# freewym/espresso

Measured on AMD Instinct MI355X. Metric: audio-hours/sec training (LibriSpeech Conformer-12 + CTC), higher is better.
Workload: dtype bf16; 1 GPU; LibriSpeech 960h Conformer-12 + CTC update step, <=26000 frames & <=24 utts per GPU, V=5004, on-GPU fbank+CMVN+SpecAugment, dropout 0.1, clip 2.0, Adam; parallelism=dp1

## Files before the change

### espresso_amd/csrc/conv_igemm.hip

```cpp
#include <hip/hip_runtime.h>

#include "gemm_common.h"

namespace {

typedef const __attribute__((address_space(1))) void* gptr_t;
typedef __attribute__((address_space(3))) void* lptr_t;

struct ConvGatherArgs {
  const bf16_t* src;
  const bf16_t* W;
  bf16_t* out;
  const float* bias;
  double* stats;
  const bf16_t* zero;
  int RB, RT, RF;
  int ST, SF, SC;
  int at, af;
  int ntaps;
  int bt[9], bf[9], koff[9];
  int N;
  long ldw;
  int OT, OF, ot_mul, ot_add, of_mul, of_add;
};

template <int BN_>
__global__ __launch_bounds__(256, 2) void conv_gather_kernel(const ConvGatherArgs a) {
  constexpr int BM_ = 128, NST = 2;
  constexpr int NJ = BN_ / 32;
  constexpr int A_BYTES = BM_ * ROW_BYTES, STAGE = A_BYTES + BN_ * ROW_BYTES;
  constexpr int NA = BM_ / 32, NB = BN_ / 32;
  extern __shared__ __attribute__((aligned(16))) char dsm[];
  const int tid = threadIdx.x, lane = tid & 63, wave = tid >> 6;
  const int wm = wave >> 1, wcol = (wave & 1) * (BN_ / 2);
  const uint32_t M = (uint32_t)a.RB * a.RT * a.RF;
  const uint32_t m0 = blockIdx.x * BM_;
  const int cpt = a.SC / BK;
  const int nk = a.ntaps * cpt;

  int rowb[NA], rowt[NA], rowf[NA];
  int cs[NA];
#pragma unroll
  for (int i = 0; i < NA; ++i) {
    const int r = (wave + 4 * i) * 8 + (lane >> 3);
    cs[i] = (lane & 7) ^ (r & 7) ^ ((r >> 4) & 7);
    const uint32_t p = m0 + r;
    if (p < M) {
      const uint32_t q = p / (uint32_t)a.RF, b = q / (uint32_t)a.RT;
      const int rf = (int)(p - q * a.RF), rt = (int)(q - b * a.RT);
      rowb[i] = (int)b * a.ST;
      rowt[i] = rt * a.at;
      rowf[i] = rf * a.af;
    } else {
      rowb[i] = -1;
      rowt[i] = rowf[i] = 0;
    }
  }
  const bf16_t* bp[NB];
#pragma unroll
  for (int i = 0; i < NB; ++i) {
    const int r = (wave + 4 * i) * 8 + (lane >> 3);
    const int c = (lane & 7) ^ (r & 7) ^ ((r >> 4) & 7);
    bp[i] = a.W + (long)min(r, a.N - 1) * a.ldw + c * 8;
  }
  auto issue = [&](int stage, int kt) {
    const int tap = kt / cpt, chunk = kt - tap * cpt;
    const int dt = a.bt[tap], df = a.bf[tap];
    const long ko = a.koff[tap] + chunk * BK;
    char* base = dsm + stage * STAGE + wave * 1024;
#pragma unroll
    for (int i = 0; i < NA; ++i) {
      const int st = rowt[i] + dt, sf = rowf[i] + df;
      const bool ok = rowb[i] >= 0 && (unsigned)st < (unsigned)a.ST && (unsigned)sf < (unsigned)a.SF;
      const bf16_t* s = ok ? a.src + (((long)(rowb[i] + st)) * a.SF + sf) * a.SC + chunk * BK + cs[i] * 8 : a.zero + cs[i] * 8;
      __builtin_amdgcn_global_load_lds((gptr_t)s, (lptr_t)(base + i * 4096), 16, 0, 0);
    }
#pragma unroll
    for (int i = 0; i < NB; ++i)
      __builtin_amdgcn_global_load_lds((gptr_t)(bp[i] + ko), (lptr_t)(base + A_BYTES + i * 4096), 16, 0, 0);
  };

  f32x4_t acc[4][NJ];
#pragma unroll
  for (int i = 0; i < 4; ++i)
#pragma unroll
    for (int j = 0; j < NJ; ++j) acc[i][j] = (f32x4_t){0.f, 0.f, 0.f, 0.f};
  uint32_t a_off[2][4], b_off[2][NJ];
#pragma unroll
  for (int ks = 0; ks < 2; ++ks) {
#pragma unroll
    for (int i = 0; i < 4; ++i) a_off[ks][i] = lds_off(wm * 64 + i * 16 + (lane & 15), ks * 4 + (lane >> 4));
#pragma unroll
    for (int j = 0; j < NJ; ++j) b_off[ks][j] = A_BYTES + lds_off(wcol + j * 16 + (lane & 15), ks * 4 + (lane >> 4));
  }

  if (nk > 0) issue(0, 0);
  int stage = 0;
  for (int kt = 0; kt < nk; ++kt) {
    asm volatile("s_waitcnt vmcnt(0)" ::: "memory");
    __builtin_amdgcn_s_barrier();
    if (kt + 1 < nk) issue(stage ^ 1, kt + 1);
    const char* st = dsm + stage * STAGE;
#pragma unroll
    for (int ks = 0; ks < 2; ++ks) {
      bf16x8_t af[4], bfr[NJ];
#pragma unroll
      for (int i = 0; i < 4; ++i) af[i] = *reinterpret_cast<const bf16x8_t*>(st + a_off[ks][i]);
#pragma unroll
      for (int j = 0; j < NJ; ++j) bfr[j] = *reinterpret_cast<const bf16x8_t*>(st + b_off[ks][j]);
#pragma unroll
      for (int i = 0; i < 4; ++i)
#pragma unroll
        for (int j = 0; j < NJ; ++j)
          acc[i][j] = __builtin_amdgcn_mfma_f32_16x16x32_bf16(
              __builtin_bit_cast(__attribute__((ext_vector_type(8))) __bf16, af[i]),
              __builtin_bit_cast(__attribute__((ext_vector_type(8))) __bf16, bfr[j]), acc[i][j], 0, 0, 0);
    }
    stage ^= 1;
  }

  constexpr int CG = BN_ / 8;
  constexpr int RL = 256 / CG;
  float* sC = reinterpret_cast<float*>(dsm);
  const int cg = tid % CG, rlane = tid / CG;
  float bias8[8], s8[8], q8[8];
#pragma unroll
  for (int e = 0; e < 8; ++e) {
    bias8[e] = a.bias ? a.bias[cg * 8 + e] : 0.f;
    s8[e] = q8[e] = 0.f;
  }
#pragma unroll 1
  for (int half = 0; half < 2; ++half) {
    __syncthreads();
    if (wm == half) {
#pragma unroll
      for (int i = 0; i < 4; ++i)
#pragma unroll
        for (int j = 0; j < NJ; ++j)
#pragma unroll
          for (int r = 0; r < 4; ++r) sC[(i * 16 + (lane >> 4) * 4 + r) * BN_ + wcol + j * 16 + (lane & 15)] = acc[i][j][r];
    }
    __syncthreads();
#pragma unroll 1
    for (int pass = 0; pass < 64 / RL; ++pass) {
      const int rl = pass * RL + rlane;
      const uint32_t p = m0 + half * 64 + rl;
      if (p < M) {
        const uint32_t q = p / (uint32_t)a.RF, b = q / (uint32_t)a.RT;
        const int rf = (int)(p - q * a.RF), rt = (int)(q - b * a.RT);
        const long orow = ((long)b * a.OT + (long)rt * a.ot_mul + a.ot_add) * a.OF + (long)rf * a.of_mul + a.of_add;
        const float4 x0 = *reinterpret_cast<const float4*>(sC + rl * BN_ + cg * 8);
        const float4 x1 = *reinterpret_cast<const float4*>(sC + rl * BN_ + cg * 8 + 4);
        float v[8] = {x0.x, x0.y, x0.z, x0.w, x1.x, x1.y, x1.z, x1.w};
#pragma unroll
        for (int e = 0; e < 8; ++e) v[e] += bias8[e];
        uint4 u;
        u.x = pack_bf2(v[0], v[1]); u.y = pack_bf2(v[2], v[3]); u.z = pack_bf2(v[4], v[5]); u.w = pack_bf2(v[6], v[7]);
        *reinterpret_cast<uint4*>(a.out + orow * a.N + cg * 8) = u;
        if (a.stats) {
          const uint32_t w[4] = {u.x, u.y, u.z, u.w};
#pragma unroll
          for (int e = 0; e < 4; ++e) {
            const float lo = __uint_as_float(w[e] << 16), hi = __uint_as_float(w[e] & 0xffff0000u);
            s8[2 * e] += lo; q8[2 * e] += lo * lo;
            s8[2 * e + 1] += hi; q8[2 * e + 1] += hi * hi;
          }
        }
      }
    }
  }
  if (a.stats) {
    __syncthreads();
    float* red = reinterpret_cast<float*>(dsm);
#pragma unroll
    for (int e = 0; e < 8; ++e) {
      red[(rlane * 2 + 0) * BN_ + cg * 8 + e] = s8[e];
      red[(rlane * 2 + 1) * BN_ + cg * 8 + e] = q8[e];
    }
    __syncthreads();
    if (tid < 2 * BN_) {
      const int which = tid / BN_, c = tid - which * BN_;
      float t = 0.f;
      for (int r = 0; r < RL; ++r) t += red[(r * 2 + which) * BN_ + c];
      atomicAdd(a.stats + which * a.N + c, (double)t);
    }
  }
}

const bf16_t* zero_line(hipStream_t stream) {
  static bf16_t* z = nullptr;
  if (!z) {
    if (hipMalloc(&z, 256) != hipSuccess) return nullptr;
    if (hipMemsetAsync(z, 0, 256, stream) != hipSuccess) return nullptr;
    hipStreamSynchronize(stream);
  }
  return z;
}

template <int BN_>
int launch_gather(const ConvGatherArgs& a, hipStream_t stream) {
  constexpr int bytes = 2 * (128 + BN_) * ROW_BYTES;
  static bool attr_ok = hipFuncSetAttribute(reinterpret_cast<const void*>(&conv_gather_kernel<BN_>),
                                            hipFuncAttributeMaxDynamicSharedMemorySize, bytes) == hipSuccess;
  if (!attr_ok) return -1;
  const long M = (long)a.RB * a.RT * a.RF;
  if (M <= 0) return 0;
  if (M >= (1L << 31) - 128) return -1;
  hipLaunchKernelGGL((conv_gather_kernel<BN_>), dim3((unsigned)((M + 127) / 128)), dim3(256), bytes, stream, a);
  return EA_CHECK_LAUNCH();
}


struct ConvWgradArgs {
  const bf16_t* X;
  const bf16_t* dZ;
  float* slab;
  const bf16_t* zero;
  int RB, RT, RF, ST, SF, Cin, Cout;
  int at, af, ntaps;
  int bt[9], bf[9];
  int chunks_per_wg;
};

__device__ __forceinline__ int tr_sw(int r) { return (r & 3) ^ ((r >> 3) & 1); }
__device__ __forceinline__ void ds_read_tr16_x8(const uint32_t (&ad)[8], uint2 (&o)[8]) {
  asm volatile(
      "ds_read_b64_tr_b16 %0, %8\n\tds_read_b64_tr_b16 %1, %9\n\tds_read_b64_tr_b16 %2, %10\n\tds_read_b64_tr_b16 %3, %11\n\t"
      "ds_read_b64_tr_b16 %4, %12\n\tds_read_b64_tr_b16 %5, %13\n\tds_read_b64_tr_b16 %6, %14\n\tds_read_b64_tr_b16 %7, %15\n\t"
      "s_waitcnt lgkmcnt(0)"
      : "=&v"(o[0]), "=&v"(o[1]), "=&v"(o[2]), "=&v"(o[3]), "=&v"(o[4]), "=&v"(o[5]), "=&v"(o[6]), "=&v"(o[7])
      : "v"(ad[0]), "v"(ad[1]), "v"(ad[2]), "v"(ad[3]), "v"(ad[4]), "v"(ad[5]), "v"(ad[6]), "v"(ad[7])
      : "memory");
}

__global__ __launch_bounds__(256, 4) void conv_wgrad_kernel(const ConvWgradArgs a) {
  constexpr int TILE = 64 * ROW_BYTES;
  constexpr int NT = 3, NBUF = 2;
  const int tap0 = (int)(blockIdx.z % 3) * 3;
  const int zsplit = (int)(blockIdx.z / 3);
  __shared__ __attribute__((aligned(16))) char lds[(2 + NBUF) * TILE];
  const int tid = threadIdx.x, lane = tid & 63, wave = tid >> 6;
  const int wr = wave >> 1, wc = wave & 1;
  const int co0 = blockIdx.x * 64, ci0 = blockIdx.y * 64;
  const long M = (long)a.RB * a.RT * a.RF;
  const long chunk0 = (long)zsplit * a.chunks_per_wg;
  long nch = (M + 63) / 64 - chunk0;
  if (nch > a.chunks_per_wg) nch = a.chunks_per_wg;
  if (nch < 0) nch = 0;

  f32x4_t acc[NT][2][2];
#pragma unroll
  for (int t = 0; t < NT; ++t)
#pragma unroll
    for (int i = 0; i < 2; ++i)
#pragma unroll
      for (int j = 0; j < 2; ++j) acc[t][i][j] = (f32x4_t){0.f, 0.f, 0.f, 0.f};

  int rr[2], cs[2];
#pragma unroll
  for (int i = 0; i < 2; ++i) {
    rr[i] = (wave + 4 * i) * 8 + (lane >> 3);
    cs[i] = (lane & 7) ^ (tr_sw(rr[i]) << 1);
  }
  int rowb[2], rowt[2], rowf[2];
  long rowp[2];
  auto decode = [&](long ch) {
#pragma unroll
    for (int i = 0; i < 2; ++i) {
      const long p = (chunk0 + ch) * 64 + rr[i];
      rowp[i] = p;
      if (p < M) {
        const uint32_t q = (uint32_t)p / (uint32_t)a.RF, b = q / (uint32_t)a.RT;
        rowb[i] = (int)b * a.ST;
        rowt[i] = (int)(q - b * a.RT) * a.at;
        rowf[i] = (int)((uint32_t)p - q * a.RF) * a.af;
      } else {
        rowb[i] = -1;
        rowt[i] = rowf[i] = 0;
      }
    }
  };
  auto issue_A = [&](int abuf) {
#pragma unroll
    for (int i = 0; i < 2; ++i) {
      const bf16_t* s = rowb[i] >= 0 ? a.dZ + rowp[i] * a.Cout + co0 + cs[i] * 8 : a.zero + cs[i] * 8;
      __builtin_amdgcn_global_load_lds((gptr_t)s, (lptr_t)(lds + abuf * TILE + (wave + 4 * i) * 1024), 16, 0, 0);
    }
  };
  auto issue_B = [&](int buf, int tap) {
#pragma unroll
    for (int i = 0; i < 2; ++i) {
      const int st = rowt[i] + a.bt[tap0 + tap], sf = rowf[i] + a.bf[tap0 + tap];
      const bool ok = rowb[i] >= 0 && (unsigned)st < (unsigned)a.ST && (unsigned)sf < (unsigned)a.SF;
      const bf16_t* s = ok ? a.X + (((long)(rowb[i] + st)) * a.SF + sf) * a.Cin + ci0 + cs[i] * 8 : a.zero + cs[i] * 8;
      __builtin_amdgcn_global_load_lds((gptr_t)s, (lptr_t)(lds + (2 + buf) * TILE + (wave + 4 * i) * 1024), 16, 0, 0);
    }
  };
  const uint32_t lds0 = (uint32_t)(uintptr_t)lds;
  auto read_frags = [&](int tile_off, int c0, uint4 (&fr)[2][2]) {
    const int g = lane >> 4, i = lane & 15;
    uint32_t ad[8];
    uint2 o[8];
#pragma unroll
    for (int ks = 0; ks < 2; ++ks)
#pragma unroll
      for (int t = 0; t < 2; ++t)
#pragma unroll
        for (int h = 0; h < 2; ++h) {
          const int r = ks * 32 + 8 * g + (i >> 2) + 4 * h;
          const int chunk = (c0 >> 4) + t;
          ad[(ks * 2 + t) * 2 + h] = lds0 + tile_off + r * ROW_BYTES + ((chunk ^ tr_sw(r)) << 5) + (i & 3) * 8;
        }
    ds_read_tr16_x8(ad, o);
#pragma unroll
    for (int ks = 0; ks < 2; ++ks)
#pragma unroll
      for (int t = 0; t < 2; ++t) fr[ks][t] = make_uint4(o[(ks * 2 + t) * 2].x, o[(ks * 2 + t) * 2].y, o[(ks * 2 + t) * 2 + 1].x, o[(ks * 2 + t) * 2 + 1].y);
  };

  const int nsteps = (int)nch * NT;
  int is = 0, itap = 0;
  long ich = 0;
  auto issue_next = [&]() {
    if (is >= nsteps) return;
    if (itap == 0) {
      decode(ich);
      issue_A((int)(ich & 1));
    }
    issue_B(is & (NBUF - 1), itap);
    ++is;
    if (++itap == NT) { itap = 0; ++ich; }
  };
  issue_next();
  uint4 fa[2][2];
  long ch = 0;
  int tap = 0;
  for (int s = 0; s < nsteps; ++s) {
    const int tap1 = tap + 1 == NT ? 0 : tap + 1;
    asm volatile("s_waitcnt vmcnt(0)" ::: "memory");
    __builtin_amdgcn_s_barrier();
    uint4 fb[2][2];
    if (tap == 0) read_frags((int)(ch & 1) * TILE, wr * 32, fa);
    read_frags((2 + (s & (NBUF - 1))) * TILE, wc * 32, fb);
    __builtin_amdgcn_sched_barrier(0);
    issue_next();
#pragma unroll
    for (int t = 0; t < NT; ++t) {
      if (t == tap) {
#pragma unroll
        for (int ks = 0; ks < 2; ++ks)
#pragma unroll
          for (int i = 0; i < 2; ++i)
#pragma unroll
            for (int j = 0; j < 2; ++j)
              acc[t][i][j] = __builtin_amdgcn_mfma_f32_16x16x32_bf16(
                  __builtin_bit_cast(__attribute__((ext_vector_type(8))) __bf16, fa[ks][i]),
                  __builtin_bit_cast(__attribute__((ext_vector_type(8))) __bf16, fb[ks][j]), acc[t][i][j], 0, 0, 0);
      }
    }
    tap = tap1;
    if (tap1 == 0) ++ch;
  }

  float* out = a.slab + (long)zsplit * a.Cout * a.ntaps * a.Cin;
#pragma unroll
  for (int t = 0; t < NT; ++t) {
    {
#pragma unroll
      for (int i = 0; i < 2; ++i)
#pragma unroll
        for (int j = 0; j < 2; ++j)
#pragma unroll
          for (int r = 0; r < 4; ++r) {
            const int co = co0 + wr * 32 + i * 16 + (lane >> 4) * 4 + r, ci = ci0 + wc * 32 + j * 16 + (lane & 15);
            out[((long)co * a.ntaps + tap0 + t) * a.Cin + ci] = acc[t][i][j][r];
          }
    }
  }
}

__global__ __launch_bounds__(256) void conv_wgrad_reduce_kernel(const float* __restrict__ slab, float* __restrict__ dW, long n, int nsplit,
                                                                int cin = 0) {
  const int zper = (nsplit + gridDim.y - 1) / gridDim.y;
  const int z0 = blockIdx.y * zper, z1 = min(nsplit, z0 + zper);
  const long i = ((long)blockIdx.x * 256 + threadIdx.x) * 4;
  if (i >= n || z0 >= z1) return;
  float4 s = *reinterpret_cast<const float4*>(slab + (long)z0 * n + i);
  for (int z = z0 + 1; z < z1; ++z) {
    const float4 x = *reinterpret_cast<const float4*>(slab + (long)z * n + i);
    s.x += x.x; s.y += x.y; s.z += x.z; s.w += x.w;
  }
  if (cin > 0) {
    const long ct = i / cin;
    const int ci = (int)(i - ct * cin), tap = (int)(ct % 9);
    const long co = ct / 9;
    float* d = dW + (co * cin + ci) * 9 + tap;
    const float v[4] = {s.x, s.y, s.z, s.w};
#pragma unroll
    for (int e = 0; e < 4; ++e) {
      if (gridDim.y == 1) d[9 * e] += v[e];
      else atomicAdd(d + 9 * e, v[e]);
    }
    return;
  }
  if (gridDim.y == 1) {
    float4 d = *reinterpret_cast<const float4*>(dW + i);
    d.x += s.x; d.y += s.y; d.z += s.z; d.w += s.w;
    *reinterpret_cast<float4*>(dW + i) = d;
  } else {
    atomicAdd(dW + i, s.x); atomicAdd(dW + i + 1, s.y); atomicAdd(dW + i + 2, s.z); atomicAdd(dW + i + 3, s.w);
  }
}

static int wgrad_split(long M, int Cin, int Cout) {
  const long chunks = (M + 63) / 64;
  const int blocks = (Cin / 64) * (Cout / 64);
  constexpr long target = 256;
  long nsplit = (target + blocks - 1) / blocks;
  if (nsplit > chunks / 8) nsplit = chunks / 8;
  if (nsplit < 1) nsplit = 1;
  return (int)nsplit;
}

}

extern "C" int ea_conv3x3_fwd(const void* X, const void* W, const float* bias, void* Z, double* stats, int B, int T, int F,
                              int Cin, int Cout, int sy, int sx, hipStream_t stream) {
  if (B <= 0 || T <= 0 || F <= 0) return 0;
  if (Cin % 64 || (Cout != 64 && Cout != 128) || sy < 1 || sx < 1) return -2;
  ConvGatherArgs a;
  a.src = (const bf16_t*)X; a.W = (const bf16_t*)W; a.out = (bf16_t*)Z; a.bias = bias; a.stats = stats;
  a.zero = zero_line(stream);
  if (!a.zero) return -1;
  const int To = (T - 1) / sy + 1, Fo = (F - 1) / sx + 1;
  a.RB = B; a.RT = To; a.RF = Fo;
  a.ST = T; a.SF = F; a.SC = Cin;
  a.at = sy; a.af = sx;
  a.ntaps = 9;
  for (int ky = 0; ky < 3; ++ky)
    for (int kx = 0; kx < 3; ++kx) {
      const int t = ky * 3 + kx;
      a.bt[t] = ky - 1; a.bf[t] = kx - 1; a.koff[t] = t * Cin;
    }
  a.N = Cout; a.ldw = 9L * Cin;
  a.OT = To; a.OF = Fo; a.ot_mul = 1; a.ot_add = 0; a.of_mul = 1; a.of_add = 0;
  return Cout == 128 ? launch_gather<128>(a, stream) : launch_gather<64>(a, stream);
}

extern "C" int ea_conv3x3_dgrad(const void* dZ, const void* Wd, void* dX, int B, int T, int F, int Cin, int Cout, int sy, int sx,
                                hipStream_t stream) {
  if (B <= 0 || T <= 0 || F <= 0) return 0;
  if (Cout % 64 || (Cin != 64 && Cin != 128) || sy < 1 || sx < 1 || sy > 2 || sx > 2) return -2;
  const int To = (T - 1) / sy + 1, Fo = (F - 1) / sx + 1;
  const bf16_t* zero = zero_line(stream);
  if (!zero) return -1;
  for (int pt = 0; pt < sy; ++pt)
    for (int pf = 0; pf < sx; ++pf) {
      ConvGatherArgs a;
      a.src = (const bf16_t*)dZ; a.W = (const bf16_t*)Wd; a.out = (bf16_t*)dX; a.bias = nullptr; a.stats = nullptr; a.zero = zero;
      a.RB = B; a.RT = (T - pt + sy - 1) / sy; a.RF = (F - pf + sx - 1) / sx;
      a.ST = To; a.SF = Fo; a.SC = Cout;
      a.at = 1; a.af = 1;
      a.ntaps = 0;
      for (int ky = 0; ky < 3; ++ky) {
        if ((pt + 1 - ky) % sy) continue;
        for (int kx = 0; kx < 3; ++kx) {
          if ((pf + 1 - kx) % sx) continue;
          const int t = a.ntaps++;
          a.bt[t] = (pt + 1 - ky) / sy; a.bf[t] = (pf + 1 - kx) / sx; a.koff[t] = (ky * 3 + kx) * Cout;
        }
      }
      a.N = Cin; a.ldw = 9L * Cout;
      a.OT = T; a.OF = F; a.ot_mul = sy; a.ot_add = pt; a.of_mul = sx; a.of_add = pf;
      if (a.RT <= 0 || a.RF <= 0) continue;
      if (a.ntaps == 0) return -2;
      const int rc = Cin == 128 ? launch_gather<128>(a, stream) : launch_gather<64>(a, stream);
      if (rc) return rc;
    }
  return 0;
}

extern "C" long ea_conv3x3_wgrad_workspace_bytes(int B, int T, int F, int Cin, int Cout, int sy, int sx) {
  const int To = (T - 1) / sy + 1, Fo = (F - 1) / sx + 1;
  return (long)wgrad_split((long)B * To * Fo, Cin, Cout) * Cout * 9 * Cin * (long)sizeof(float);
}

static int conv3x3_wgrad_impl(const void* X, const void* dZ, float* dW, void* workspace, int B, int T, int F, int Cin, int Cout,
                              int sy, int sx, int param_layout, hipStream_t stream);
extern "C" int ea_conv3x3_wgrad(const void* X, const void* dZ, float* dW, void* workspace, int B, int T, int F, int Cin, int Cout,
                                int sy, int sx, hipStream_t stream) {
  return conv3x3_wgrad_impl(X, dZ, dW, workspace, B, T, F, Cin, Cout, sy, sx, 0, stream);
}
extern "C" int ea_conv3x3_wgrad_param_layout(const void* X, const void* dZ, float* dW, void* workspace, int B, int T, int F, int Cin,
                                             int Cout, int sy, int sx, hipStream_t stream) {
  return conv3x3_wgrad_impl(X, dZ, dW, workspace, B, T, F, Cin, Cout, sy, sx, 1, stream);
}
static int conv3x3_wgrad_impl(const void* X, const void* dZ, float* dW, void* workspace, int B, int T, int F, int Cin, int Cout,
                              int sy, int sx, int param_layout, hipStream_t stream) {
  if (B <= 0 || T <= 0 || F <= 0) return 0;
  if (Cin % 64 || Cout % 64 || sy < 1 || sx < 1 || !workspace) return -2;
  ConvWgradArgs a;
  a.X = (const bf16_t*)X; a.dZ = (const bf16_t*)dZ; a.slab = (float*)workspace;
  a.zero = zero_line(stream);
  if (!a.zero) return -1;
  const int To = (T - 1) / sy + 1, Fo = (F - 1) / sx + 1;
  a.RB = B; a.RT = To; a.RF = Fo; a.ST = T; a.SF = F; a.Cin = Cin; a.Cout = Cout;
  a.at = sy; a.af = sx; a.ntaps = 9;
  for (int ky = 0; ky < 3; ++ky)
    for (int kx = 0; kx < 3; ++kx) { a.bt[ky * 3 + kx] = ky - 1; a.bf[ky * 3 + kx] = kx - 1; }
  const long M = (long)B * To * Fo;
  if (M >= (1L << 31) - 128) return -2;
  const int nsplit = wgrad_split(M, Cin, Cout);
  const long chunks = (M + 63) / 64;
  a.chunks_per_wg = (int)((chunks + nsplit - 1) / nsplit);
  hipLaunchKernelGGL(conv_wgrad_kernel, dim3(Cout / 64, Cin / 64, nsplit * 3), dim3(256), 0, stream, a);
  const long n = (long)Cout * 9 * Cin;
  const long blocks = (n / 4 + 255) / 256;
  int zg = (int)(1024 / blocks);
  if (zg > nsplit / 4) zg = nsplit / 4;
  if (zg < 1) zg = 1;
  hipLaunchKernelGGL(conv_wgrad_reduce_kernel, dim3((unsigned)blocks, zg), dim3(256), 0, stream, (const float*)workspace, dW, n, nsplit,
                     param_layout ? Cin : 0);
  return EA_CHECK_LAUNCH();
}
```

Before: 5.328 audio-hours/sec.

## Pipeline conv gather kernel with multi-stage ring and precomputed tap validity masks

Reworks the implicit-GEMM conv gather kernel's main loop. Fragments for the next k-slice are read from LDS while the current MFMAs run, and the wait on global loads becomes a partial vmcnt instead of a full drain. Per-row base pointers and a tap-validity bitmask are precomputed, so the per-step index math becomes a readlane plus a bit test. Wave count and stage count become template parameters, but the defaults stay at 4 waves and 2 stages, so only the scheduling and address changes take effect. This adds code complexity and register pressure, which may hurt occupancy.

```diff
diff --git a/espresso_amd/csrc/conv_igemm.hip b/espresso_amd/csrc/conv_igemm.hip
--- a/espresso_amd/csrc/conv_igemm.hip
+++ b/espresso_amd/csrc/conv_igemm.hip
@@ -24,12 +24,20 @@
   int OT, OF, ot_mul, ot_add, of_mul, of_add;
 };
 
-template <int BN_>
-__global__ __launch_bounds__(256, 2) void conv_gather_kernel(const ConvGatherArgs a) {
-  constexpr int BM_ = 128, NST = 2;
+template <int N>
+__device__ __forceinline__ void wait_vmcnt() {
+  static_assert(N >= 0 && N < 64, "vmcnt is a 6-bit counter");
+  asm volatile("s_waitcnt vmcnt(%0)" ::"n"(N) : "memory");
+}
+
+template <int BN_, int NW_, int NST_>
+__global__ __launch_bounds__(NW_ * 64, 2) void conv_gather_kernel(const ConvGatherArgs a) {
+  static_assert(NST_ >= 2 && NST_ <= 4 && (NW_ == 4 || NW_ == 8) && BN_ % (8 * NW_) == 0, "ring of two to four stages, 4 or 8 wavefronts");
+  constexpr int BM_ = 32 * NW_, NT = 64 * NW_;
   constexpr int NJ = BN_ / 32;
   constexpr int A_BYTES = BM_ * ROW_BYTES, STAGE = A_BYTES + BN_ * ROW_BYTES;
-  constexpr int NA = BM_ / 32, NB = BN_ / 32;
+  constexpr int NA = BM_ / (8 * NW_), NB = BN_ / (8 * NW_);
+  constexpr int L = NA + NB;
   extern __shared__ __attribute__((aligned(16))) char dsm[];
   const int tid = threadIdx.x, lane = tid & 63, wave = tid >> 6;
   const int wm = wave >> 1, wcol = (wave & 1) * (BN_ / 2);
@@ -38,46 +46,57 @@
   const int cpt = a.SC / BK;
   const int nk = a.ntaps * cpt;
 
-  int rowb[NA], rowt[NA], rowf[NA];
-  int cs[NA];
+  const bf16_t* ap[NA];
+  uint32_t avalid[NA];
 #pragma unroll
   for (int i = 0; i < NA; ++i) {
-    const int r = (wave + 4 * i) * 8 + (lane >> 3);
-    cs[i] = (lane & 7) ^ (r & 7) ^ ((r >> 4) & 7);
+    const int r = (wave + NW_ * i) * 8 + (lane >> 3);
+    const int cs = (lane & 7) ^ (r & 7) ^ ((r >> 4) & 7);
     const uint32_t p = m0 + r;
-    if (p < M) {
-      const uint32_t q = p / (uint32_t)a.RF, b = q / (uint32_t)a.RT;
-      const int rf = (int)(p - q * a.RF), rt = (int)(q - b * a.RT);
-      rowb[i] = (int)b * a.ST;
-      rowt[i] = rt * a.at;
-      rowf[i] = rf * a.af;
-    } else {
-      rowb[i] = -1;
-      rowt[i] = rowf[i] = 0;
-    }
-  }
+    const uint32_t q = p / (uint32_t)a.RF, b = q / (uint32_t)a.RT;
+    const int st0 = (int)(q - b * a.RT) * a.at, sf0 = (int)(p - q * a.RF) * a.af;
+    ap[i] = a.src + (((long)b * a.ST + st0) * a.SF + sf0) * a.SC + cs * 8;
+    uint32_t v = 0;
+#pragma unroll
+    for (int t = 0; t < 9; ++t) {
+      const int st = st0 + a.bt[t], sf = sf0 + a.bf[t];
+      if (t < a.ntaps && p < M && (unsigned)st < (unsigned)a.ST && (unsigned)sf < (unsigned)a.SF) v |= 1u << t;
+    }
+    avalid[i] = v;
+  }
+  const bf16_t* zp = a.zero + (lane & 7) * 8;
   const bf16_t* bp[NB];
 #pragma unroll
   for (int i = 0; i < NB; ++i) {
-    const int r = (wave + 4 * i) * 8 + (lane >> 3);
+    const int r = (wave + NW_ * i) * 8 + (lane >> 3);
     const int c = (lane & 7) ^ (r & 7) ^ ((r >> 4) & 7);
     bp[i] = a.W + (long)min(r, a.N - 1) * a.ldw + c * 8;
   }
-  auto issue = [&](int stage, int kt) {
-    const int tap = kt / cpt, chunk = kt - tap * cpt;
-    const int dt = a.bt[tap], df = a.bf[tap];
-    const long ko = a.koff[tap] + chunk * BK;
+  int tap_src = 0, tap_k = 0;
+#pragma unroll
+  for (int t = 0; t < 9; ++t) {
+    const int ts = (a.bt[t] * a.SF + a.bf[t]) * a.SC, tk = a.koff[t];
+    tap_src = lane == t ? ts : tap_src;
+    tap_k = lane == t ? tk : tap_k;
+  }
+  int itap = 0, ichunk = 0;
+  auto issue = [&](int stage) {
+    const long so = __builtin_amdgcn_readlane(tap_src, itap) + ichunk * BK;
+    const long ko = __builtin_amdgcn_readlane(tap_k, itap) + ichunk * BK;
+    const uint32_t bit = 1u << itap;
     char* base = dsm + stage * STAGE + wave * 1024;
 #pragma unroll
     for (int i = 0; i < NA; ++i) {
-      const int st = rowt[i] + dt, sf = rowf[i] + df;
-      const bool ok = rowb[i] >= 0 && (unsigned)st < (unsigned)a.ST && (unsigned)sf < (unsigned)a.SF;
-      const bf16_t* s = ok ? a.src + (((long)(rowb[i] + st)) * a.SF + sf) * a.SC + chunk * BK + cs[i] * 8 : a.zero + cs[i] * 8;
-      __builtin_amdgcn_global_load_lds((gptr_t)s, (lptr_t)(base + i * 4096), 16, 0, 0);
+      const bf16_t* s = (avalid[i] & bit) ? ap[i] + so : zp;
+      __builtin_amdgcn_global_load_lds((gptr_t)s, (lptr_t)(base + i * (NW_ * 1024)), 16, 0, 0);
     }
 #pragma unroll
     for (int i = 0; i < NB; ++i)
-      __builtin_amdgcn_global_load_lds((gptr_t)(bp[i] + ko), (lptr_t)(base + A_BYTES + i * 4096), 16, 0, 0);
+      __builtin_amdgcn_global_load_lds((gptr_t)(bp[i] + ko), (lptr_t)(base + A_BYTES + i * (NW_ * 1024)), 16, 0, 0);
+    if (++ichunk == cpt) {
+      ichunk = 0;
+      ++itap;
+    }
   };
 
   f32x4_t acc[4][NJ];
@@ -93,34 +112,67 @@
 #pragma unroll
     for (int j = 0; j < NJ; ++j) b_off[ks][j] = A_BYTES + lds_off(wcol + j * 16 + (lane & 15), ks * 4 + (lane >> 4));
   }
-
-  if (nk > 0) issue(0, 0);
+  struct Frags {
+    bf16x8_t af[4], bfr[NJ];
+  };
+  auto read_frags = [&](Frags& f, int stage, int ks) {
+    const char* st = dsm + stage * STAGE;
+#pragma unroll
+    for (int i = 0; i < 4; ++i) f.af[i] = *reinterpret_cast<const bf16x8_t*>(st + a_off[ks][i]);
+#pragma unroll
+    for (int j = 0; j < NJ; ++j) f.bfr[j] = *reinterpret_cast<const bf16x8_t*>(st + b_off[ks][j]);
+    __builtin_amdgcn_sched_barrier(0);
+  };
+  auto mfma_frags = [&](const Frags& f) {
+#pragma unroll
+    for (int i = 0; i < 4; ++i)
+#pragma unroll
+      for (int j = 0; j < NJ; ++j)
+        acc[i][j] = __builtin_amdgcn_mfma_f32_16x16x32_bf16(
+            __builtin_bit_cast(__attribute__((ext_vector_type(8))) __bf16, f.af[i]),
+            __builtin_bit_cast(__attribute__((ext_vector_type(8))) __bf16, f.bfr[j]), acc[i][j], 0, 0, 0);
+  };
+  auto wait_steps = [&](int younger) {
+    if constexpr (NST_ >= 4)
+      if (younger >= 3) return wait_vmcnt<3 * L>();
+    if constexpr (NST_ >= 3)
+      if (younger >= 2) return wait_vmcnt<2 * L>();
+    if (younger >= 1) return wait_vmcnt<L>();
+    wait_vmcnt<0>();
+  };
+
+#pragma unroll
+  for (int s = 0; s < NST_; ++s)
+    if (s < nk) issue(s);
+  auto lds_reads_done = [&]() {
+    __builtin_amdgcn_sched_barrier(0);
+    __builtin_amdgcn_s_waitcnt(0xc07f);
+  };
+  Frags f0, f1;
+  if (nk > 0) {
+    wait_steps(min(nk, NST_) - 1);
+    __builtin_amdgcn_s_barrier();
+    read_frags(f0, 0, 0);
+    lds_reads_done();
+  }
   int stage = 0;
   for (int kt = 0; kt < nk; ++kt) {
-    asm volatile("s_waitcnt vmcnt(0)" ::: "memory");
-    __builtin_amdgcn_s_barrier();
-    if (kt + 1 < nk) issue(stage ^ 1, kt + 1);
-    const char* st = dsm + stage * STAGE;
-#pragma unroll
-    for (int ks = 0; ks < 2; ++ks) {
-      bf16x8_t af[4], bfr[NJ];
-#pragma unroll
-      for (int i = 0; i < 4; ++i) af[i] = *reinterpret_cast<const bf16x8_t*>(st + a_off[ks][i]);
-#pragma unroll
-      for (int j = 0; j < NJ; ++j) bfr[j] = *reinterpret_cast<const bf16x8_t*>(st + b_off[ks][j]);
-#pragma unroll
-      for (int i = 0; i < 4; ++i)
-#pragma unroll
-        for (int j = 0; j < NJ; ++j)
-          acc[i][j] = __builtin_amdgcn_mfma_f32_16x16x32_bf16(
-              __builtin_bit_cast(__attribute__((ext_vector_type(8))) __bf16, af[i]),
-              __builtin_bit_cast(__attribute__((ext_vector_type(8))) __bf16, bfr[j]), acc[i][j], 0, 0, 0);
-    }
-    stage ^= 1;
+    read_frags(f1, stage, 1);
+    mfma_frags(f0);
+    lds_reads_done();
+    if (kt + 1 < nk) {
+      wait_steps(min(nk - kt - 2, NST_ - 2));
+      __builtin_amdgcn_s_barrier();
+      if (kt + NST_ < nk) issue(stage);
+      stage = stage + 1 == NST_ ? 0 : stage + 1;
+      read_frags(f0, stage, 0);
+    }
+    mfma_frags(f1);
+    lds_reads_done();
   }
 
   constexpr int CG = BN_ / 8;
-  constexpr int RL = 256 / CG;
+  constexpr int RL = NT / CG;
   float* sC = reinterpret_cast<float*>(dsm);
   const int cg = tid % CG, rlane = tid / CG;
   float bias8[8], s8[8], q8[8];
@@ -130,7 +182,7 @@
     s8[e] = q8[e] = 0.f;
   }
 #pragma unroll 1
-  for (int half = 0; half < 2; ++half) {
+  for (int half = 0; half < BM_ / 64; ++half) {
     __syncthreads();
     if (wm == half) {
 #pragma unroll
@@ -197,16 +249,20 @@
   return z;
 }
 
+constexpr int CG64_NW = 4, CG64_NST = 2;
+constexpr int CG128_NW = 4, CG128_NST = 2;
+
 template <int BN_>
 int launch_gather(const ConvGatherArgs& a, hipStream_t stream) {
-  constexpr int bytes = 2 * (128 + BN_) * ROW_BYTES;
-  static bool attr_ok = hipFuncSetAttribute(reinterpret_cast<const void*>(&conv_gather_kernel<BN_>),
+  constexpr int NW = BN_ == 128 ? CG128_NW : CG64_NW, NST = BN_ == 128 ? CG128_NST : CG64_NST;
+  constexpr int BM = 32 * NW, bytes = NST * (BM + BN_) * ROW_BYTES;
+  static bool attr_ok = hipFuncSetAttribute(reinterpret_cast<const void*>(&conv_gather_kernel<BN_, NW, NST>),
                                             hipFuncAttributeMaxDynamicSharedMemorySize, bytes) == hipSuccess;
   if (!attr_ok) return -1;
   const long M = (long)a.RB * a.RT * a.RF;
   if (M <= 0) return 0;
-  if (M >= (1L << 31) - 128) return -1;
-  hipLaunchKernelGGL((conv_gather_kernel<BN_>), dim3((unsigned)((M + 127) / 128)), dim3(256), bytes, stream, a);
+  if (M >= (1L << 31) - BM) return -1;
+  hipLaunchKernelGGL((conv_gather_kernel<BN_, NW, NST>), dim3((unsigned)((M + BM - 1) / BM)), dim3(NW * 64), bytes, stream, a);
   return EA_CHECK_LAUNCH();
 }
 
```

Result: no change. 5.328 audio-hours/sec (-0.0%).
